# facebookresearch/nonrigid_nerf

Hardware: NVIDIA H100
Metric: rays/sec (64c+128f samples, 8x256 MLP), example_sequence training step (higher is better)
Workload: dtype f16 (tensor-core operands; f32 accumulate)

## Files before the change

include/nrnerf_b200.h:

```cpp
#ifndef NRNERF_B200_H
#define NRNERF_B200_H

#include <stddef.h>
#include <stdint.h>

#ifdef __cplusplus
extern "C" {
#endif

#define NRN_ABI_VERSION 4

#define NRN_OK 0
#define NRN_E_INVALID (-1)
#define NRN_E_CUDA (-2)
#define NRN_E_DEVICE (-3)

int nrn_abi_version(void);
const char* nrn_last_error(void);

int nrn_device_error(int* code_out);

size_t nrn_packed_nerf_bytes(void);
size_t nrn_packed_bender_bytes(void);
int nrn_pack_nerf(const float* const* w, const float* const* b, int input_ch, int out_ch, void* packed,
// ... 23 lines not shown
  const void* nerf_packed;
  const void* bender_packed;
  int32_t out_ch;
  int32_t use_cutoff;  float rigidity_cutoff;
  int32_t use_scaling; float scaling;
  int32_t use_removal; float removal_threshold;
  float* raw;
  float* initial_input_pts;
  float* input_pts;
  float* unmasked_offsets;
  float* masked_offsets;
  float* rigidity_mask;
  void* stash;
  void* stream;
  void* relu_mask;
} NrnFieldArgs;
int nrn_field_forward(const NrnFieldArgs* args);

typedef struct NrnCompositeArgs {
  const float* raw;
  const float* z_vals;
  const float* rays_d;
  int32_t rays_d_stride;
  const float* noise;
  int32_t n_rays, n_samples, channels, white_bkgd;
  float* rgb_map;
  float* disp_map;
  float* acc_map;
  float* depth_map;
  float* weights;
// ... 282 lines not shown
```

nonrigid_nerf_b200/_lib.py:

```python
from __future__ import annotations

import ctypes as C
import os
import threading

_HERE = os.path.dirname(os.path.abspath(__file__))
LIB_PATH = os.path.join(_HERE, "libnrnerf_b200.so")
ABI_VERSION = 4

_f32p = C.POINTER(C.c_float)
_vp = C.c_void_p


class NrnFieldArgs(C.Structure):
    _fields_ = [
        ("rays", _vp), ("z_vals", _vp), ("points", _vp), ("points_stride", C.c_int64),
        ("latents", _vp), ("latent_stride", C.c_int64),
        ("n_rays", C.c_int32), ("n_samples", C.c_int32),
        ("nerf_packed", _vp), ("bender_packed", _vp),
        ("out_ch", C.c_int32),
        ("use_cutoff", C.c_int32), ("rigidity_cutoff", C.c_float),
        ("use_scaling", C.c_int32), ("scaling", C.c_float),
        ("use_removal", C.c_int32), ("removal_threshold", C.c_float),
        ("raw", _vp), ("initial_input_pts", _vp), ("input_pts", _vp), ("unmasked_offsets", _vp),
        ("masked_offsets", _vp), ("rigidity_mask", _vp),
        ("stash", _vp),
        ("stream", _vp),
        ("relu_mask", _vp),
    ]


class NrnViewArgs(C.Structure):
    _fields_ = [
        ("views_packed", _vp), ("viewdirs", _vp), ("viewdirs_stride", C.c_int64), ("workspace", _vp),
    ]


class NrnViewTrainArgs(C.Structure):
    _fields_ = [("views_stash", _vp), ("hv_mask", _vp)]


class NrnViewBwdArgs(C.Structure):
    _fields_ = [("views_t_packed", _vp), ("views_stash", _vp), ("views_grad_stash", _vp), ("hv_mask", _vp)]
# ... 211 lines not shown
    "nrn_lpips": (C.c_int, [C.POINTER(NrnLpipsArgs)]),
    "nrn_timing_enable": (C.c_int, [C.c_int]),
    "nrn_timing_read": (C.c_int, [C.POINTER(C.c_double), C.POINTER(C.c_int), C.c_int]),
}

KERNEL_KINDS = ("field_fwd", "field_dgrad", "wgrad", "composite", "composite_bwd", "divergence")
TC_KERNEL_KINDS = ("tc_latent_bias", "tc_latent_bwd")
VIEW_KERNEL_KINDS = ("views_bend", "views_field")
VIEW_TRAIN_KERNEL_KINDS = ("views_field_train", "views_dgrad", "views_wgrad")
DET_KERNEL_KINDS = ("latent_reduce", "div_loss_reduce")
HELD_OUT_KERNEL_KINDS = ("field_dgrad_held_out", "div_bwd_held_out")
EVAL_KERNEL_KINDS = ("image_scores", "disparity_images", "frame_std_image")
FRAME_IMAGE_KERNEL_KINDS = ("frame_images",)
MESH_KERNEL_KINDS = ("mesh_points", "mesh_count", "mesh_emit", "mesh_colors")
LPIPS_KERNEL_KINDS = ("lpips_input", "lpips_conv", "lpips_pool", "lpips_distance")


def timing_enable(on: bool) -> None:
    check(load().nrn_timing_enable(1 if on else 0), "timing_enable")


def timing_read(kinds=KERNEL_KINDS):
    n = len(kinds)
    ms = (C.c_double * n)()
    cnt = (C.c_int * n)()
    check(load().nrn_timing_read(ms, cnt, n), "timing_read")
    return {k: (ms[i], cnt[i]) for i, k in enumerate(kinds)}

_lib = None
_lock = threading.Lock()
# ... 35 lines not shown
```

nonrigid_nerf_b200/csrc/c_abi.cu:

```cuda
#include <cstdarg>
#include <cstdio>
#include <cstring>
#include <cstdlib>
#include "../../include/nrnerf_b200.h"
#include "nrn_common.cuh"
#include "pack.cuh"
#include "ray_ops.cuh"
#include "wgrad.cuh"
#include "div.cuh"
#include "loss.cuh"
#include "adam.cuh"
#include "peer.cuh"
#include "det_reduce.cuh"
#include "eval.cuh"
#include "mesh.cuh"
#include "lpips.cuh"

namespace nrn {
cudaError_t launch_field_fwd(const FieldFwdParams& p, bool has_bender, int num_sms, cudaStream_t stream);
cudaError_t launch_field_bwd(const FieldBwdParams& p, bool has_bender, int num_sms, cudaStream_t stream);
cudaError_t launch_field_bwd_det(const FieldBwdParams& p, float* latent_rows, int num_sms, cudaStream_t stream);
cudaError_t launch_field_bwd_held(const FieldBwdParams& p, float* latent_rows, const uint8_t* held, int num_sms, cudaStream_t stream);
cudaError_t launch_field_fwd_tc(const FieldFwdParams& p, int num_sms, cudaStream_t stream);
cudaError_t launch_tc_latent_bias(const float* lat, long long lat_stride, int n_rays, const float* w0, const float* b0, const float* w5,
                                  const float* b5, float* rb, cudaStream_t stream);
cudaError_t launch_tc_latent_bwd(const TcBwdParams& p, cudaStream_t stream);
cudaError_t launch_field_bend(const FieldFwdParams& p, const ViewParams& v, int num_sms, cudaStream_t stream);
cudaError_t launch_field_views(const FieldFwdParams& p, const ViewParams& v, int num_sms, cudaStream_t stream);
cudaError_t launch_field_views_train(const FieldFwdParams& p, const ViewParams& v, const ViewTrainParams& t, int num_sms, cudaStream_t stream);
cudaError_t launch_field_bwd_views(const FieldBwdParams& p, const ViewBwdParams& v, int num_sms, cudaStream_t stream);
}

namespace {

thread_local char g_err[512] = "";

int fail(int code, const char* fmt, ...) {
  va_list ap;
  va_start(ap, fmt);
  vsnprintf(g_err, sizeof(g_err), fmt, ap);
  va_end(ap);
  return code;
}
int cuda_fail(cudaError_t e, const char* what) {
  return fail(NRN_E_CUDA, "%s: %s", what, cudaGetErrorString(e));
}

constexpr int kMaxDevices = 64;
struct DeviceState {
  int* err_word = nullptr;
  int num_sms = 0;
};
DeviceState g_dev[kMaxDevices];

int device_state(DeviceState** out) {
  int dev = 0;
  cudaError_t e = cudaGetDevice(&dev);
  if (e != cudaSuccess) return cuda_fail(e, "cudaGetDevice");
  if (dev < 0 || dev >= kMaxDevices) return fail(NRN_E_INVALID, "device index %d out of range", dev);
  DeviceState& s = g_dev[dev];
  if (!s.err_word) {
    cudaDeviceProp prop;
    e = cudaGetDeviceProperties(&prop, dev);
    if (e != cudaSuccess) return cuda_fail(e, "cudaGetDeviceProperties");
    if (prop.major != 9 || prop.minor != 0)
      return fail(NRN_E_INVALID, "nrnerf_b200 is built for sm_90a (H100) only, found sm_%d%d", prop.major, prop.minor);
// ... 241 lines not shown
  if (!pix || !poses || !K || !rays_o || !rays_d || (images && !target)) return fail(NRN_E_INVALID, "nrn_ray_batch: null argument");
  static_assert(sizeof(long long) == sizeof(int64_t), "int64");
  const cudaError_t e = nrn::launch_ray_batch(reinterpret_cast<const long long*>(pix), n, poses, K, image_to_view, images, H, W, rays_o, rays_d,
                                              target, static_cast<cudaStream_t>(stream));
  return e == cudaSuccess ? NRN_OK : cuda_fail(e, "ray_batch_kernel");
}

int nrn_median_visibility_index(const float* weights, int n_rays, int n_samples, int64_t* index, void* stream) {
  if (n_rays < 0 || n_samples < 1) return fail(NRN_E_INVALID, "nrn_median_visibility_index: bad sizes");
  if (n_rays == 0) return NRN_OK;
  if (!weights || !index) return fail(NRN_E_INVALID, "nrn_median_visibility_index: null argument");
  const cudaError_t e = nrn::launch_median_index(weights, n_rays, n_samples, reinterpret_cast<long long*>(index), static_cast<cudaStream_t>(stream));
  return e == cudaSuccess ? NRN_OK : cuda_fail(e, "median_index_kernel");
}

static int field_forward(const NrnFieldArgs* a, const float* ray_bias, const char* who) {
  long long P;
  int tiles;
  int rc = check_field_args(a, who, &P, &tiles);
  if (rc || P == 0) return rc;
  if (!a->raw) return fail(NRN_E_INVALID, "%s: null argument", who);
  if (a->points && a->n_samples != 1) return fail(NRN_E_INVALID, "%s: point mode needs n_samples=1, stride>=3", who);
  DeviceState* ds;
  rc = device_state(&ds);
  if (rc) return rc;
  nrn::FieldFwdParams p = field_fwd_params(a, P, tiles, ds->err_word);
  p.ray_bias = ray_bias; p.ray_bias_stride = a->latent_stride == 0 ? 0 : 2 * 256;
  cudaStream_t st = static_cast<cudaStream_t>(a->stream);
  if (ray_bias) return timed(0, st, "field_fwd_tc_kernel", [&] { return nrn::launch_field_fwd_tc(p, ds->num_sms, st); });
  return timed(0, st, "field_fwd_kernel", [&] { return nrn::launch_field_fwd(p, a->bender_packed != nullptr, ds->num_sms, st); });
}

int nrn_field_forward(const NrnFieldArgs* a) { return field_forward(a, nullptr, "nrn_field_forward"); }

int nrn_field_forward_tc(const NrnFieldArgs* a, const float* ray_bias) {
  if (!a) return fail(NRN_E_INVALID, "nrn_field_forward_tc: null args");
  if (a->bender_packed) return fail(NRN_E_INVALID, "nrn_field_forward_tc: the time-conditioned baseline has no bender (bender_packed must be NULL)");
  if (a->latent_stride < 0) return fail(NRN_E_INVALID, "nrn_field_forward_tc: latent_stride < 0");
  if (a->n_rays > 0 && !ray_bias) return fail(NRN_E_INVALID, "nrn_field_forward_tc: null ray_bias (nrn_tc_latent_bias output)");
  return field_forward(a, ray_bias, "nrn_field_forward_tc");
}

size_t nrn_packed_views_bytes(void) { return nrn::kViewsPackedBytes; }

// ... 36 lines not shown
  if (bend && (!v->workspace || !aligned16(v->workspace)))
    return fail(NRN_E_INVALID, "%s: a bender needs the workspace (nrn_views_workspace_bytes, 16-byte aligned)", who);
  if (v->views_packed && !aligned16(v->views_packed)) return fail(NRN_E_INVALID, "%s: packed weights must be 16-byte aligned", who);
  DeviceState* ds;
  rc = device_state(&ds);
  if (rc) return rc;
  cudaStream_t st = static_cast<cudaStream_t>(a->stream);
  nrn::FieldFwdParams p = field_fwd_params(a, P, tiles, ds->err_word);
  nrn::ViewParams vp{};
  const uint8_t* vw = static_cast<const uint8_t*>(v->views_packed);
  vp.w = vw; vp.bias = vw ? reinterpret_cast<const float*>(vw + nrn::kViewsWBytes) : nullptr;
  vp.viewdirs = v->viewdirs; vp.viewdirs_stride = v->viewdirs_stride;
  if (bend) {
    nrn::FieldFwdParams b = p;
    if (a->points) { b.n_rays = static_cast<int>(P); b.S = 1; }
    vp.ws = static_cast<float4*>(v->workspace);
    rc = timed(8, st, "field_bend_kernel", [&] { return nrn::launch_field_bend(b, vp, ds->num_sms, st); });
    if (rc || !a->raw) return rc;
    p.d_init = p.d_bent = nullptr;
  }
  return timed(9, st, "field_views_kernel", [&] { return nrn::launch_field_views(p, vp, ds->num_sms, st); });
}

size_t nrn_packed_views_t_bytes(void) { return nrn::kViewsTWBytes; }

int nrn_pack_views_t(const float* const* w, void* packed, void* stream) {
  if (!w || !packed) return fail(NRN_E_INVALID, "nrn_pack_views_t: null argument");
  if (!aligned16(packed)) return fail(NRN_E_INVALID, "nrn_pack_views_t: packed buffer must be 16-byte aligned");
  nrn::ViewsSrc src{};
  for (int i = 0; i < 3; ++i) {
    if (!w[i]) return fail(NRN_E_INVALID, "nrn_pack_views_t: null layer %d", i);
    src.w[i] = w[i];
// ... 841 lines not shown
```

nonrigid_nerf_b200/csrc/field_fwd.cu:

```cuda
#include "field_mma.cuh"

namespace nrn {

namespace {

constexpr int kFwdStageLd = 12;
constexpr int kFwdHBytes = kStHb1.chunks * kChunkBytes;
static_assert(kStHb2.chunks <= kStHb1.chunks && kStHb3.chunks <= kStHb1.chunks && kStHb4.chunks <= kStHb1.chunks, "bender images fit H");
constexpr int kFwdRingStages = 5;
constexpr size_t kFwdSmemBytes = kFwdHBytes + kEBytes + kFwdRingStages * kRingStageBytes + 2 * kWgRows * kFwdStageLd * sizeof(float) +
                                 sizeof(RingShared<kFwdRingStages>) + 64;
static_assert(kFwdSmemBytes <= 227 * 1024, "forward kernel: dynamic shared memory per block");

static_assert(fwd::step(fwd::L2) == fwd::step(fwd::L1) && fwd::step(fwd::L3) == fwd::step(fwd::L1) &&
              fwd::step(fwd::L4) == fwd::step(fwd::L1) && fwd::step(fwd::L6) == fwd::step(fwd::L1) &&
              fwd::step(fwd::L7) == fwd::step(fwd::L1), "step_at: one default shape");
__device__ __forceinline__ Step step_at(int step) {
  switch (step) {
    case fwd::B0: return step_imm<fwd::B0>();
    case fwd::B1: return step_imm<fwd::B1>();
    case fwd::B2: return step_imm<fwd::B2>();
    case fwd::B3: return step_imm<fwd::B3>();
    case fwd::B4: return step_imm<fwd::B4>();
    case fwd::L0: return step_imm<fwd::L0>();
    case fwd::L5: return step_imm<fwd::L5>();
    case fwd::Head: return step_imm<fwd::Head>();
    default: return step_imm<fwd::L1>();
  }
}
template <int NCOLS, bool MASK, int NR>
__device__ __forceinline__ void epi_bias_relu_store(const float (&acc)[NR], const float* __restrict__ bias, uint8_t* img, int g,
                                                    uint8_t* mask_tile, int mask_off) {
  const int r0 = g * kWgRows + acc_r0(), q = acc_q();
  ReluMask<NCOLS> m;
  if constexpr (MASK) m.clear();
#pragma unroll
  for (int j = 0; j < NCOLS / 8; ++j) {
    const float2 b = __ldg(reinterpret_cast<const float2*>(bias + 8 * j + 2 * q));
// ... 85 lines not shown
}

static_assert(views::step(views::Feature) == fwd::step(fwd::L1), "step_at_views: Feature has the trunk's shape");
__device__ __forceinline__ Step step_at_views(int step) {
  switch (step) {
    case fwd::L0: return step_imm<fwd::L0>();
    case fwd::L5: return step_imm<fwd::L5>();
    case fwd::Head: return step_imm<fwd::Head>();
    case views::ViewsE: return step_imm<views::ViewsE>();
    case views::ViewsF: return step_imm<views::ViewsF>();
    case views::Rgb: return step_imm<views::Rgb>();
    default: return step_imm<fwd::L1>();
  }
}

enum Part : int { kFull, kBend, kViews };

}

template <bool HAS_BENDER, bool TRAIN, bool LATENT_BIAS, int PART = kFull>
__device__ __forceinline__ void field_fwd_body(const FieldFwdParams& p, const ViewParams& v = ViewParams{},
                                               const ViewTrainParams& t = ViewTrainParams{}) {
  static_assert(!(HAS_BENDER && LATENT_BIAS), "the time-conditioned baseline has no bender");
  static_assert(PART == kFull || (!LATENT_BIAS && (PART == kBend) == HAS_BENDER && (!TRAIN || PART == kViews)),
                "view-head parts: inference, or training of the view-head kernel without a bender");
  constexpr int kHBytes = PART == kViews ? 0 : kFwdHBytes;
  extern __shared__ __align__(1024) uint8_t smem[];
  uint8_t* act = smem;
  uint8_t* ring_buf = smem + kHBytes + kEBytes;
  float* stage_all = reinterpret_cast<float*>(ring_buf + kFwdRingStages * kRingStageBytes);
  auto* sh = reinterpret_cast<RingShared<kFwdRingStages>*>(stage_all + 2 * kWgRows * kFwdStageLd);

  const int warp = threadIdx.x >> 5;
  const int lane = threadIdx.x & 31;

  if (threadIdx.x == 0) sh->init();
  __syncthreads();
  const Waiter W{&sh->abort_flag, p.err};
  Ring<kFwdRingStages> ring{ring_buf, sh->w_full, sh->w_empty};

  if (warp >= 8) {
    setmaxnreg_dec<kProducerRegs>();
    if (warp == 8 && lane == 0) {
      if constexpr (PART == kViews) produce(p.nerf_w, v.w, p.n_tiles, fwd::L0, views::kEnd, views::Feature, step_at_views, ring, W);
      else produce(p.bend_w, p.nerf_w, p.n_tiles, HAS_BENDER ? fwd::B0 : fwd::L0, PART == kBend ? fwd::L0 : fwd::kCount, fwd::L0, step_at, ring, W);
    }
    return;
  }

  setmaxnreg_inc<kConsumerRegs>();
  const int g = warp >> 2;
  const int tw = threadIdx.x & 127;
  const bool row_thread = tw < kWgRows;
  const int bar = 1 + g;
  const bool wg_leader = tw == 0;
  uint8_t* Hs = act;
  uint8_t* Es = act + kHBytes;
  uint8_t* e_row = Es + (g * kWgRows + tw) * 16;
  const uint32_t a_h = smem_u32(Hs) + g * kWgRows * 16;
  const uint32_t a_e = smem_u32(Es) + g * kWgRows * 16;
  float* stg = stage_all + g * kWgRows * kFwdStageLd;
  float* my_stg = stg + tw * kFwdStageLd;

  for (int tile = blockIdx.x; tile < p.n_tiles; tile += gridDim.x) {
    const long long pt = static_cast<long long>(tile) * kTileM + g * kWgRows + tw;
    const bool valid = row_thread && pt < p.P;
    uint8_t* st = p.stash ? p.stash + static_cast<long long>(tile) * kStashTileBytes : nullptr;
    const StashWriter<true> sw{st, wg_leader, bar, g};
    uint8_t* mk = TRAIN ? p.relu_mask + static_cast<long long>(tile) * kMaskTileBytes : nullptr;
    float x[3] = {0.f, 0.f, 0.f};
    long long ray = 0;
    if (valid) {
      ray = pt / p.S;
      if (PART == kViews && v.ws) {
        const float4 q = __ldg(v.ws + pt);
        const bool first = pt % p.S == 0;
        const float4 o = __ldg(v.ws + (first ? pt + 1 : pt - 1));
        x[0] = q.x; x[1] = q.y; x[2] = q.z;
        const float dx = first ? o.x - q.x : q.x - o.x, dy = first ? o.y - q.y : q.y - o.y, dz = first ? o.z - q.z : q.z - o.z;
        const float nrm = __fadd_rn(__fsqrt_rn(__fadd_rn(__fadd_rn(__fmul_rn(dx, dx), __fmul_rn(dy, dy)), __fmul_rn(dz, dz))), 1e-6f);
        my_stg[8] = __fdiv_rn(dx, nrm); my_stg[9] = __fdiv_rn(dy, nrm); my_stg[10] = __fdiv_rn(dz, nrm);
        my_stg[11] = q.w;
      } else if (p.pts) {
        const float* q = p.pts + pt * p.pts_stride;
        x[0] = __ldg(q + 0); x[1] = __ldg(q + 1); x[2] = __ldg(q + 2);
      } else {
        const float z = __ldg(p.z_vals + pt);
        const float* r = p.rays + ray * 8;
        x[0] = __fadd_rn(__ldg(r + 0), __fmul_rn(__ldg(r + 3), z));
        x[1] = __fadd_rn(__ldg(r + 1), __fmul_rn(__ldg(r + 4), z));
        x[2] = __fadd_rn(__ldg(r + 2), __fmul_rn(__ldg(r + 5), z));
      }
      if (PART == kViews && !v.ws) {
        const float* vd = v.viewdirs + (p.pts ? pt : ray) * v.viewdirs_stride;
        my_stg[8] = __ldg(vd + 0); my_stg[9] = __ldg(vd + 1); my_stg[10] = __ldg(vd + 2);
      }
      if (p.d_init) {
        p.d_init[pt * 3 + 0] = x[0]; p.d_init[pt * 3 + 1] = x[1]; p.d_init[pt * 3 + 2] = x[2];
      }
    }
    float rigidity = 0.f;
    if (HAS_BENDER) {
      sw.begin();
      if (row_thread) {
        float in[48];
#pragma unroll
        for (int d = 0; d < 3; ++d) {
          const float hi = __half2float(__float2half_rn(x[d]));
          in[d] = hi;
          in[3 + d] = x[d] - hi;
        }
        const float* lat = p.latents + ray * p.latent_stride;
#pragma unroll
        for (int i = 0; i < kLatent; ++i) in[6 + i] = valid ? __ldg(lat + i) : 0.f;
#pragma unroll
        for (int i = 38; i < 48; ++i) in[i] = 0.f;
        pack_row(in, e_row);
      }
      sw.ready(kStBin, Es);
      {
        Acc<fwd::B0> acc;
        wg_gemm_step<fwd::B0>(acc, ring, [&](uint32_t) { return a_e; }, W, 301);
        sw.begin();
        epi_bias_relu_store<kMkHb1.cols, TRAIN>(acc, p.bend_bias + fwd::b_off(fwd::B0), Hs, g, mk, kMkHb1.off);
        sw.ready(kStHb1, Hs);
        wg_gemm_step<fwd::B1>(acc, ring, [&](uint32_t) { return a_h; }, W, 302);
        sw.begin();
        epi_bias_relu_store<kMkHb2.cols, TRAIN>(acc, p.bend_bias + fwd::b_off(fwd::B1), Hs, g, mk, kMkHb2.off);
        sw.ready(kStHb2, Hs);
      }
      {
        Acc<fwd::B2> acc;
        wg_gemm_step<fwd::B2>(acc, ring, [&](uint32_t) { return a_h; }, W, 303);
        sw.begin();
        epi_bias_relu_store<kMkHb3.cols, TRAIN>(acc, p.bend_bias + fwd::b_off(fwd::B2), Hs, g, mk, kMkHb3.off);
        if (acc_q() == 0) {
          stg[acc_r0() * kFwdStageLd] = acc[32];
          stg[(acc_r0() + 8) * kFwdStageLd] = acc[34];
        }
        sw.ready(kStHb3, Hs);
        if (row_thread) {
          const float rr = my_stg[0] + __ldg(p.bend_bias + fwd::b_off(fwd::B2) + 64);
          rigidity = (tanhf(rr) + 1.0f) * 0.5f;
          if (p.use_cutoff && rigidity <= p.cutoff) rigidity = 0.f;
        }
      }
      {
        Acc<fwd::B3> acc;
        wg_gemm_step<fwd::B3>(acc, ring, [&](uint32_t) { return a_h; }, W, 304);
        sw.begin();
        epi_bias_relu_store<kMkHb4.cols, TRAIN>(acc, p.bend_bias + fwd::b_off(fwd::B3), Hs, g, mk, kMkHb4.off);
        sw.ready(kStHb4, Hs);
      }
      {
        Acc<fwd::B4> acc;
        wg_gemm_step<fwd::B4>(acc, ring, [&](uint32_t) { return a_h; }, W, 305);
        stage_cols<0, 1>(acc, stg, kFwdStageLd);
        wg_bar(bar);
        if (row_thread) {
          float un[3], ma[3];
#pragma unroll
          for (int d = 0; d < 3; ++d) {
            un[d] = my_stg[d];
            ma[d] = __fmul_rn(rigidity, un[d]);
            if (p.use_scaling) ma[d] = __fmul_rn(ma[d], p.scaling);
          }
          if (valid) {
            if (p.d_unmasked) { p.d_unmasked[pt * 3 + 0] = un[0]; p.d_unmasked[pt * 3 + 1] = un[1]; p.d_unmasked[pt * 3 + 2] = un[2]; }
            if (p.d_masked) { p.d_masked[pt * 3 + 0] = ma[0]; p.d_masked[pt * 3 + 1] = ma[1]; p.d_masked[pt * 3 + 2] = ma[2]; }
            if (p.d_rigid) p.d_rigid[pt] = rigidity;
          }
#pragma unroll
          for (int d = 0; d < 3; ++d) x[d] = __fadd_rn(x[d], ma[d]);
        }
      }
    }
    if (valid && p.d_bent) {
      p.d_bent[pt * 3 + 0] = x[0]; p.d_bent[pt * 3 + 1] = x[1]; p.d_bent[pt * 3 + 2] = x[2];
    }
    if constexpr (PART == kBend) {
      if (valid) v.ws[pt] = make_float4(x[0], x[1], x[2], rigidity);
      continue;
    }
    sw.begin();
    if (row_thread) write_pe(x, e_row);
    sw.ready(kStE, Es);
    uint32_t h[kMaskHCols / 16][4];
    int ray_r0 = 0, ray_r8 = 0;
    if constexpr (LATENT_BIAS) {
      const long long r0 = static_cast<long long>(tile) * kTileM + g * kWgRows + acc_r0();
      ray_r0 = static_cast<int>(min(r0, p.P - 1) / p.S);
      ray_r8 = static_cast<int>(min(r0 + 8, p.P - 1) / p.S);
    }
#pragma unroll 1
    for (int L = 0; L < 8; ++L) {
      Acc<fwd::L1> acc;
      if (L == 0) wg_gemm_step<fwd::L0>(acc, ring, [&](uint32_t) { return a_e; }, W, 310);
// ... 6 lines not shown
        epi_bias_frag<kMaskHCols, true, TRAIN>(acc, p.nerf_bias + L * fwd::b_off(fwd::L1), h, st + st_h(L + 1).off, g,
                                               mk + kMkH + L * kMaskHBytes);
      }
    }
    if constexpr (PART == kViews) {
      uint8_t* vst = TRAIN ? t.vstash + static_cast<long long>(tile) * kVStashTileBytes : nullptr;
      const StashWriter<true> vsw{vst, wg_leader, bar, g};
      {
        Acc<fwd::Head> acc;
        wg_gemm_rs<fwd::step(fwd::Head).N, fwd::step(fwd::Head).k16>(acc, h, ring, false, 0u, W, 320);
        stage_cols<0, 1>(acc, stg, kFwdStageLd);
        if constexpr (TRAIN) sw.begin();
        else wg_bar(bar);
        if (row_thread) {
          float alpha = my_stg[3] + __ldg(p.nerf_bias + fwd::b_off(fwd::Head) + 3);
          if (v.ws && p.use_removal && my_stg[11] >= p.removal) alpha *= 0.f;
          const bool dir_ok = !TRAIN || valid;
          const float d[3] = {dir_ok ? my_stg[8] : 0.f, dir_ok ? my_stg[9] : 0.f, dir_ok ? my_stg[10] : 0.f};
          my_stg[11] = alpha;
          write_dir_enc(d, e_row);
        }
      }
      {
        Acc<views::Feature> acc;
        wg_gemm_rs<views::step(views::Feature).N, views::step(views::Feature).k16>(acc, h, ring, false, 0u, W, 330);
        epi_bias_frag<256, false, TRAIN>(acc, v.bias + views::b_off(views::Feature), h, TRAIN ? vst + kVsF.off : nullptr, g);
      }
      if constexpr (TRAIN) {
        vsw.ready(kVsDir, Es);
      } else {
        fence_proxy_async_smem();
// ... 26 lines not shown
      stage_cols<0, 1>(acc, stg, kFwdStageLd);
      wg_bar(bar);
      if (valid) {
        float o[5];
#pragma unroll
        for (int c = 0; c < 5; ++c) o[c] = my_stg[c] + __ldg(p.nerf_bias + fwd::b_off(fwd::Head) + c);
        if (HAS_BENDER && p.use_removal && rigidity >= p.removal) o[3] *= 0.f;
        float* dst = p.raw + pt * p.out_ch;
        for (int c = 0; c < p.out_ch; ++c) dst[c] = o[c];
      }
    }
  }
  if (p.stash && wg_leader) tma_bulk_wait<0>();
}

template <bool HAS_BENDER, bool TRAIN>
__global__ void __launch_bounds__(kFwdThreads, 1) field_fwd_kernel(const FieldFwdParams p) { field_fwd_body<HAS_BENDER, TRAIN, false>(p); }
template <bool TRAIN>
__global__ void __launch_bounds__(kFwdThreads, 1) field_fwd_tc_kernel(const FieldFwdParams p) { field_fwd_body<false, TRAIN, true>(p); }
__global__ void __launch_bounds__(kFwdThreads, 1) field_bend_kernel(const FieldFwdParams p, const ViewParams v) {
  field_fwd_body<true, false, false, kBend>(p, v);
}
__global__ void __launch_bounds__(kFwdThreads, 1) field_views_kernel(const FieldFwdParams p, const ViewParams v) {
  field_fwd_body<false, false, false, kViews>(p, v);
}
__global__ void __launch_bounds__(kFwdThreads, 1) field_views_train_kernel(const FieldFwdParams p, const ViewParams v, const ViewTrainParams t) {
  field_fwd_body<false, true, false, kViews>(p, v, t);
}

constexpr int kTcRaysPerBlock = 16;
__global__ void __launch_bounds__(256) tc_latent_bias_kernel(const float* __restrict__ lat, long long lat_stride, int n_rays,
                                                             const float* __restrict__ w0, const float* __restrict__ b0,
                                                             const float* __restrict__ w5, const float* __restrict__ b5,
                                                             float* __restrict__ rb) {
  __shared__ float zs[kTcRaysPerBlock][kLatent];
  const int o = threadIdx.x;
  const int n0 = blockIdx.x * kTcRaysPerBlock;
// ... 19 lines not shown
    float* dst = rb + static_cast<long long>(n0 + i) * 512;
    dst[o] = ba + sa;
    dst[256 + o] = bb + sb;
  }
}

size_t field_fwd_smem_bytes() { return kFwdSmemBytes; }

cudaError_t launch_field_fwd(const FieldFwdParams& p, bool has_bender, int num_sms, cudaStream_t stream) {
  const size_t smem = field_fwd_smem_bytes();
  const bool train = p.relu_mask != nullptr;
  if (has_bender) return launch_field(train ? field_fwd_kernel<true, true> : field_fwd_kernel<true, false>, p, num_sms, smem, stream);
  return launch_field(train ? field_fwd_kernel<false, true> : field_fwd_kernel<false, false>, p, num_sms, smem, stream);
}

size_t field_views_smem_bytes() { return kFwdSmemBytes - kFwdHBytes; }

cudaError_t launch_field_bend(const FieldFwdParams& p, const ViewParams& v, int num_sms, cudaStream_t stream) {
  return launch_field(field_bend_kernel, p, num_sms, field_fwd_smem_bytes(), stream, v);
}

cudaError_t launch_field_views(const FieldFwdParams& p, const ViewParams& v, int num_sms, cudaStream_t stream) {
  return launch_field(field_views_kernel, p, num_sms, field_views_smem_bytes(), stream, v);
}

cudaError_t launch_field_views_train(const FieldFwdParams& p, const ViewParams& v, const ViewTrainParams& t, int num_sms, cudaStream_t stream) {
  return launch_field(field_views_train_kernel, p, num_sms, field_views_smem_bytes(), stream, v, t);
}

cudaError_t launch_field_fwd_tc(const FieldFwdParams& p, int num_sms, cudaStream_t stream) {
  const bool train = p.relu_mask != nullptr;
  return launch_field(train ? field_fwd_tc_kernel<true> : field_fwd_tc_kernel<false>, p, num_sms, field_fwd_smem_bytes(), stream);
}

cudaError_t launch_tc_latent_bias(const float* lat, long long lat_stride, int n_rays, const float* w0, const float* b0, const float* w5,
                                  const float* b5, float* rb, cudaStream_t stream) {
  tc_latent_bias_kernel<<<(n_rays + kTcRaysPerBlock - 1) / kTcRaysPerBlock, 256, 0, stream>>>(lat, lat_stride, n_rays, w0, b0, w5, b5, rb);
  return cudaGetLastError();
}

}
```

nonrigid_nerf_b200/csrc/nrn_common.cuh:

```cuda
#pragma once
#include <cuda_runtime.h>
#include <stdint.h>

namespace nrn {

constexpr int kTileM = 128;
constexpr int kChunkBytes = kTileM * 16;
constexpr int kRingStageBytes = 32768;
constexpr int kFwdThreads = 384;
constexpr int kProducerRegs = 40, kConsumerRegs = 232;
constexpr int kLatent = 32;

struct WImage {
  int rows, chunks;
  __host__ __device__ constexpr int bytes() const { return rows * chunks * 16; }
  __host__ __device__ constexpr WImage t() const { return {8 * chunks, rows / 8}; }
};

namespace fwd {
enum Id : int { B0, B1, B2, B3, B4, L0, L1, L2, L3, L4, L5, L6, L7, Head, kCount };
__host__ __device__ constexpr WImage image(int s) {
  switch (s) {
    case B0: return {96, 6};
    case B1: return {96, 12};
// ... 206 lines not shown
  const float* bend_bias;
  float cutoff, scaling, removal;
  int use_cutoff, use_scaling, use_removal;
  int out_ch;
  float* raw;
  float* d_init;
  float* d_bent;
  float* d_unmasked;
  float* d_masked;
  float* d_rigid;
  uint8_t* stash;
  int* err;
  uint8_t* relu_mask;
  const float* ray_bias;
  long long ray_bias_stride;
};

struct ViewParams {
  const uint8_t* w;
  const float* bias;
  const float* viewdirs;
  long long viewdirs_stride;
  float4* ws;
};
struct ViewTrainParams {
  uint8_t* vstash;
  uint8_t* hv_mask;
};
struct ViewBwdParams {
  const uint8_t* wT;
  const uint8_t* hv_mask;
  uint8_t* vgstash;
};

struct TcBwdParams {
  const uint8_t* gstash;
  const float* amax;
  long long P;
// ... 12 lines not shown
```

nonrigid_nerf_b200/ops.py:

```python
from __future__ import annotations

import ctypes as C
from typing import Dict, Optional, Tuple

import torch

from . import _lib

LATENT = 32
FORCE_PACK = False


def _ptr(t: Optional[torch.Tensor]):
    return None if t is None else C.c_void_p(t.data_ptr())


def _stream():
    return C.c_void_p(torch.cuda.current_stream().cuda_stream)


def _f32c(t: torch.Tensor, name: str) -> torch.Tensor:
    if not t.is_cuda:
        raise RuntimeError(f"nonrigid_nerf_b200: {name} must be a CUDA tensor (there is no CPU path)")
    if t.dtype != torch.float32:
# ... 219 lines not shown
        viewdirs = viewdirs.reshape(viewdirs.shape[0], -1).float().contiguous().to(dev)
    return viewdirs, viewdirs.stride(0) if viewdirs.shape[0] > 1 else 3


def _field(rays, z_vals, points, latents, nerf_pack, bender_pack, out_ch, cutoff, scaling, removal, want_details, stash=None, relu_mask=None,
           tc_net=None):
    tc = tc_net if bender_pack is None else None
    if latents is None and (bender_pack is not None or tc is not None):
        raise RuntimeError("nonrigid_nerf_b200: " + ("ray bending" if tc is None else "time_conditioned_baseline") + " needs latents")
    a, raw, details, keep = _field_args(rays, z_vals, points, 1, latents if bender_pack is not None or tc is not None else None, nerf_pack,
                                        bender_pack, out_ch, (cutoff, scaling, removal), True, want_details)
    if stash is not None:
        a.stash = stash.data_ptr()
    if relu_mask is not None:
        a.relu_mask = relu_mask.data_ptr()
    with torch.cuda.device(keep[0].device):
        if tc is not None:
            ray_bias = tc_ray_bias(tc, keep[-1], a.latent_stride)
            _lib.check(_lib.load().nrn_field_forward_tc(C.byref(a), _ptr(ray_bias)), "field_forward_tc")
        else:
            _lib.check(_lib.load().nrn_field_forward(C.byref(a)), "field_forward")
    return raw, details


def field_forward(rays: torch.Tensor, z_vals: torch.Tensor, latents: Optional[torch.Tensor], nerf_pack: torch.Tensor,
                  bender_pack: Optional[torch.Tensor], out_ch: int, cutoff: Optional[float] = None,
                  scaling: Optional[float] = None, removal: Optional[float] = None,
                  want_details: bool = False, stash: Optional[torch.Tensor] = None,
                  relu_mask: Optional[torch.Tensor] = None, tc_net=None) -> Tuple[torch.Tensor, Dict[str, torch.Tensor]]:
    return _field(rays, z_vals, None, latents, nerf_pack, bender_pack, out_ch, cutoff, scaling, removal, want_details, stash,
# ... 191 lines not shown
```

Baseline: 492,500.

## Split ray bender into a standalone kernel with smem-resident weights

The forward field kernel used to run the bender MLP inline before the NeRF MLP, streaming bender weights through the shared weight ring and reserving an extra activation buffer. A new dedicated bend kernel now loads all bender weights into shared memory once per CTA via TMA, runs four warpgroups (two tiles per CTA) with double-buffered activation images, and writes bent points and rigidity to a float4 workspace. The main forward kernel then reads that workspace, which frees its H buffer in shared memory. The cost is an extra kernel launch, a global round trip of P float4s, and a workspace allocation on each Python call.

```diff
diff --git a/include/nrnerf_b200.h b/include/nrnerf_b200.h
--- a/include/nrnerf_b200.h
+++ b/include/nrnerf_b200.h
@@ -61,6 +61,7 @@
   void* stash;
   void* stream;
   void* relu_mask;
+  void* workspace;
 } NrnFieldArgs;
 int nrn_field_forward(const NrnFieldArgs* args);
 
diff --git a/nonrigid_nerf_b200/_lib.py b/nonrigid_nerf_b200/_lib.py
--- a/nonrigid_nerf_b200/_lib.py
+++ b/nonrigid_nerf_b200/_lib.py
@@ -26,7 +26,7 @@
         ("masked_offsets", _vp), ("rigidity_mask", _vp),
         ("stash", _vp),
         ("stream", _vp),
-        ("relu_mask", _vp),
+        ("relu_mask", _vp), ("workspace", _vp),
     ]
 
 
@@ -268,6 +268,7 @@
 FRAME_IMAGE_KERNEL_KINDS = ("frame_images",)
 MESH_KERNEL_KINDS = ("mesh_points", "mesh_count", "mesh_emit", "mesh_colors")
 LPIPS_KERNEL_KINDS = ("lpips_input", "lpips_conv", "lpips_pool", "lpips_distance")
+BEND_KERNEL_KINDS = ("field_bend",)
 
 
 def timing_enable(on: bool) -> None:
diff --git a/nonrigid_nerf_b200/csrc/c_abi.cu b/nonrigid_nerf_b200/csrc/c_abi.cu
--- a/nonrigid_nerf_b200/csrc/c_abi.cu
+++ b/nonrigid_nerf_b200/csrc/c_abi.cu
@@ -25,7 +25,7 @@
 cudaError_t launch_tc_latent_bias(const float* lat, long long lat_stride, int n_rays, const float* w0, const float* b0, const float* w5,
                                   const float* b5, float* rb, cudaStream_t stream);
 cudaError_t launch_tc_latent_bwd(const TcBwdParams& p, cudaStream_t stream);
-cudaError_t launch_field_bend(const FieldFwdParams& p, const ViewParams& v, int num_sms, cudaStream_t stream);
+cudaError_t launch_field_bend(const FieldFwdParams& p, int num_sms, cudaStream_t stream);
 cudaError_t launch_field_views(const FieldFwdParams& p, const ViewParams& v, int num_sms, cudaStream_t stream);
 cudaError_t launch_field_views_train(const FieldFwdParams& p, const ViewParams& v, const ViewTrainParams& t, int num_sms, cudaStream_t stream);
 cudaError_t launch_field_bwd_views(const FieldBwdParams& p, const ViewBwdParams& v, int num_sms, cudaStream_t stream);
@@ -50,6 +50,8 @@
 struct DeviceState {
   int* err_word = nullptr;
   int num_sms = 0;
+  void* bend_ws = nullptr;
+  size_t bend_ws_bytes = 0;
 };
 DeviceState g_dev[kMaxDevices];
 
@@ -321,6 +323,32 @@
   return e == cudaSuccess ? NRN_OK : cuda_fail(e, "median_index_kernel");
 }
 
+static int bend_workspace(void* given, long long P, DeviceState* ds, cudaStream_t st, const char* who, float4** out) {
+  if (given) {
+    if (!aligned16(given)) return fail(NRN_E_INVALID, "%s: workspace must be 16-byte aligned", who);
+    *out = static_cast<float4*>(given);
+    return NRN_OK;
+  }
+  const size_t need = static_cast<size_t>(P) * sizeof(float4);
+  if (ds->bend_ws_bytes < need) {
+    cudaStreamCaptureStatus cs = cudaStreamCaptureStatusNone;
+    cudaStreamIsCapturing(st, &cs);
+    if (cs != cudaStreamCaptureStatusNone)
+      return fail(NRN_E_INVALID, "%s: a bender needs a workspace during stream capture (nrn_views_workspace_bytes)", who);
+    if (ds->bend_ws) {
+      const cudaError_t e = cudaFree(ds->bend_ws);
+      if (e != cudaSuccess) return cuda_fail(e, "cudaFree(bend workspace)");
+      ds->bend_ws = nullptr;
+      ds->bend_ws_bytes = 0;
+    }
+    const cudaError_t e = cudaMalloc(&ds->bend_ws, need);
+    if (e != cudaSuccess) return cuda_fail(e, "cudaMalloc(bend workspace)");
+    ds->bend_ws_bytes = need;
+  }
+  *out = static_cast<float4*>(ds->bend_ws);
+  return NRN_OK;
+}
+
 static int field_forward(const NrnFieldArgs* a, const float* ray_bias, const char* who) {
   long long P;
   int tiles;
@@ -335,6 +363,13 @@
   p.ray_bias = ray_bias; p.ray_bias_stride = a->latent_stride == 0 ? 0 : 2 * 256;
   cudaStream_t st = static_cast<cudaStream_t>(a->stream);
   if (ray_bias) return timed(0, st, "field_fwd_tc_kernel", [&] { return nrn::launch_field_fwd_tc(p, ds->num_sms, st); });
+  if (a->bender_packed) {
+    rc = bend_workspace(a->workspace, P, ds, st, who, &p.ws);
+    if (rc) return rc;
+    rc = timed(29, st, "field_bend_kernel", [&] { return nrn::launch_field_bend(p, ds->num_sms, st); });
+    if (rc) return rc;
+    p.d_init = p.d_bent = nullptr;
+  }
   return timed(0, st, "field_fwd_kernel", [&] { return nrn::launch_field_fwd(p, a->bender_packed != nullptr, ds->num_sms, st); });
 }
 
@@ -401,8 +436,8 @@
   if (bend) {
     nrn::FieldFwdParams b = p;
     if (a->points) { b.n_rays = static_cast<int>(P); b.S = 1; }
-    vp.ws = static_cast<float4*>(v->workspace);
-    rc = timed(8, st, "field_bend_kernel", [&] { return nrn::launch_field_bend(b, vp, ds->num_sms, st); });
+    b.ws = p.ws = static_cast<float4*>(v->workspace);
+    rc = timed(8, st, "field_bend_kernel", [&] { return nrn::launch_field_bend(b, ds->num_sms, st); });
     if (rc || !a->raw) return rc;
     p.d_init = p.d_bent = nullptr;
   }
diff --git a/nonrigid_nerf_b200/csrc/field_fwd.cu b/nonrigid_nerf_b200/csrc/field_fwd.cu
--- a/nonrigid_nerf_b200/csrc/field_fwd.cu
+++ b/nonrigid_nerf_b200/csrc/field_fwd.cu
@@ -5,10 +5,8 @@
 namespace {
 
 constexpr int kFwdStageLd = 12;
-constexpr int kFwdHBytes = kStHb1.chunks * kChunkBytes;
-static_assert(kStHb2.chunks <= kStHb1.chunks && kStHb3.chunks <= kStHb1.chunks && kStHb4.chunks <= kStHb1.chunks, "bender images fit H");
 constexpr int kFwdRingStages = 5;
-constexpr size_t kFwdSmemBytes = kFwdHBytes + kEBytes + kFwdRingStages * kRingStageBytes + 2 * kWgRows * kFwdStageLd * sizeof(float) +
+constexpr size_t kFwdSmemBytes = kEBytes + kFwdRingStages * kRingStageBytes + 2 * kWgRows * kFwdStageLd * sizeof(float) +
                                  sizeof(RingShared<kFwdRingStages>) + 64;
 static_assert(kFwdSmemBytes <= 227 * 1024, "forward kernel: dynamic shared memory per block");
 
@@ -17,11 +15,6 @@
               fwd::step(fwd::L7) == fwd::step(fwd::L1), "step_at: one default shape");
 __device__ __forceinline__ Step step_at(int step) {
   switch (step) {
-    case fwd::B0: return step_imm<fwd::B0>();
-    case fwd::B1: return step_imm<fwd::B1>();
-    case fwd::B2: return step_imm<fwd::B2>();
-    case fwd::B3: return step_imm<fwd::B3>();
-    case fwd::B4: return step_imm<fwd::B4>();
     case fwd::L0: return step_imm<fwd::L0>();
     case fwd::L5: return step_imm<fwd::L5>();
     case fwd::Head: return step_imm<fwd::Head>();
@@ -137,7 +130,20 @@
   }
 }
 
-enum Part : int { kFull, kBend, kViews };
+__device__ __forceinline__ void sample_point(const FieldFwdParams& p, long long pt, long long ray, float (&x)[3]) {
+  if (p.pts) {
+    const float* q = p.pts + pt * p.pts_stride;
+    x[0] = __ldg(q + 0); x[1] = __ldg(q + 1); x[2] = __ldg(q + 2);
+  } else {
+    const float z = __ldg(p.z_vals + pt);
+    const float* r = p.rays + ray * 8;
+    x[0] = __fadd_rn(__ldg(r + 0), __fmul_rn(__ldg(r + 3), z));
+    x[1] = __fadd_rn(__ldg(r + 1), __fmul_rn(__ldg(r + 4), z));
+    x[2] = __fadd_rn(__ldg(r + 2), __fmul_rn(__ldg(r + 5), z));
+  }
+}
+
+enum Part : int { kFull, kViews };
 
 }
 
@@ -145,12 +151,10 @@
 __device__ __forceinline__ void field_fwd_body(const FieldFwdParams& p, const ViewParams& v = ViewParams{},
                                                const ViewTrainParams& t = ViewTrainParams{}) {
   static_assert(!(HAS_BENDER && LATENT_BIAS), "the time-conditioned baseline has no bender");
-  static_assert(PART == kFull || (!LATENT_BIAS && (PART == kBend) == HAS_BENDER && (!TRAIN || PART == kViews)),
-                "view-head parts: inference, or training of the view-head kernel without a bender");
-  constexpr int kHBytes = PART == kViews ? 0 : kFwdHBytes;
+  static_assert(PART == kFull || (!LATENT_BIAS && !HAS_BENDER), "view-head kernel: no time conditioning, points from p.ws");
   extern __shared__ __align__(1024) uint8_t smem[];
   uint8_t* act = smem;
-  uint8_t* ring_buf = smem + kHBytes + kEBytes;
+  uint8_t* ring_buf = smem + kEBytes;
   float* stage_all = reinterpret_cast<float*>(ring_buf + kFwdRingStages * kRingStageBytes);
   auto* sh = reinterpret_cast<RingShared<kFwdRingStages>*>(stage_all + 2 * kWgRows * kFwdStageLd);
 
@@ -166,7 +170,7 @@
     setmaxnreg_dec<kProducerRegs>();
     if (warp == 8 && lane == 0) {
       if constexpr (PART == kViews) produce(p.nerf_w, v.w, p.n_tiles, fwd::L0, views::kEnd, views::Feature, step_at_views, ring, W);
-      else produce(p.bend_w, p.nerf_w, p.n_tiles, HAS_BENDER ? fwd::B0 : fwd::L0, PART == kBend ? fwd::L0 : fwd::kCount, fwd::L0, step_at, ring, W);
+      else produce(p.nerf_w, p.nerf_w, p.n_tiles, fwd::L0, fwd::kCount, fwd::L0, step_at, ring, W);
     }
     return;
   }
@@ -177,10 +181,8 @@
   const bool row_thread = tw < kWgRows;
   const int bar = 1 + g;
   const bool wg_leader = tw == 0;
-  uint8_t* Hs = act;
-  uint8_t* Es = act + kHBytes;
+  uint8_t* Es = act;
   uint8_t* e_row = Es + (g * kWgRows + tw) * 16;
-  const uint32_t a_h = smem_u32(Hs) + g * kWgRows * 16;
   const uint32_t a_e = smem_u32(Es) + g * kWgRows * 16;
   float* stg = stage_all + g * kWgRows * kFwdStageLd;
   float* my_stg = stg + tw * kFwdStageLd;
@@ -192,29 +194,27 @@
     const StashWriter<true> sw{st, wg_leader, bar, g};
     uint8_t* mk = TRAIN ? p.relu_mask + static_cast<long long>(tile) * kMaskTileBytes : nullptr;
     float x[3] = {0.f, 0.f, 0.f};
+    float rigidity = 0.f;
     long long ray = 0;
     if (valid) {
       ray = pt / p.S;
-      if (PART == kViews && v.ws) {
-        const float4 q = __ldg(v.ws + pt);
+      if (HAS_BENDER) {
+        const float4 q = __ldg(p.ws + pt);
+        x[0] = q.x; x[1] = q.y; x[2] = q.z;
+        rigidity = q.w;
+      } else if (PART == kViews && p.ws) {
+        const float4 q = __ldg(p.ws + pt);
         const bool first = pt % p.S == 0;
-        const float4 o = __ldg(v.ws + (first ? pt + 1 : pt - 1));
+        const float4 o = __ldg(p.ws + (first ? pt + 1 : pt - 1));
         x[0] = q.x; x[1] = q.y; x[2] = q.z;
         const float dx = first ? o.x - q.x : q.x - o.x, dy = first ? o.y - q.y : q.y - o.y, dz = first ? o.z - q.z : q.z - o.z;
         const float nrm = __fadd_rn(__fsqrt_rn(__fadd_rn(__fadd_rn(__fmul_rn(dx, dx), __fmul_rn(dy, dy)), __fmul_rn(dz, dz))), 1e-6f);
         my_stg[8] = __fdiv_rn(dx, nrm); my_stg[9] = __fdiv_rn(dy, nrm); my_stg[10] = __fdiv_rn(dz, nrm);
         my_stg[11] = q.w;
-      } else if (p.pts) {
-        const float* q = p.pts + pt * p.pts_stride;
-        x[0] = __ldg(q + 0); x[1] = __ldg(q + 1); x[2] = __ldg(q + 2);
       } else {
-        const float z = __ldg(p.z_vals + pt);
-        const float* r = p.rays + ray * 8;
-        x[0] = __fadd_rn(__ldg(r + 0), __fmul_rn(__ldg(r + 3), z));
-        x[1] = __fadd_rn(__ldg(r + 1), __fmul_rn(__ldg(r + 4), z));
-        x[2] = __fadd_rn(__ldg(r + 2), __fmul_rn(__ldg(r + 5), z));
-      }
-      if (PART == kViews && !v.ws) {
+        sample_point(p, pt, ray, x);
+      }
+      if (PART == kViews && !p.ws) {
         const float* vd = v.viewdirs + (p.pts ? pt : ray) * v.viewdirs_stride;
         my_stg[8] = __ldg(vd + 0); my_stg[9] = __ldg(vd + 1); my_stg[10] = __ldg(vd + 2);
       }
@@ -222,88 +222,8 @@
         p.d_init[pt * 3 + 0] = x[0]; p.d_init[pt * 3 + 1] = x[1]; p.d_init[pt * 3 + 2] = x[2];
       }
     }
-    float rigidity = 0.f;
-    if (HAS_BENDER) {
-      sw.begin();
-      if (row_thread) {
-        float in[48];
-#pragma unroll
-        for (int d = 0; d < 3; ++d) {
-          const float hi = __half2float(__float2half_rn(x[d]));
-          in[d] = hi;
-          in[3 + d] = x[d] - hi;
-        }
-        const float* lat = p.latents + ray * p.latent_stride;
-#pragma unroll
-        for (int i = 0; i < kLatent; ++i) in[6 + i] = valid ? __ldg(lat + i) : 0.f;
-#pragma unroll
-        for (int i = 38; i < 48; ++i) in[i] = 0.f;
-        pack_row(in, e_row);
-      }
-      sw.ready(kStBin, Es);
-      {
-        Acc<fwd::B0> acc;
-        wg_gemm_step<fwd::B0>(acc, ring, [&](uint32_t) { return a_e; }, W, 301);
-        sw.begin();
-        epi_bias_relu_store<kMkHb1.cols, TRAIN>(acc, p.bend_bias + fwd::b_off(fwd::B0), Hs, g, mk, kMkHb1.off);
-        sw.ready(kStHb1, Hs);
-        wg_gemm_step<fwd::B1>(acc, ring, [&](uint32_t) { return a_h; }, W, 302);
-        sw.begin();
-        epi_bias_relu_store<kMkHb2.cols, TRAIN>(acc, p.bend_bias + fwd::b_off(fwd::B1), Hs, g, mk, kMkHb2.off);
-        sw.ready(kStHb2, Hs);
-      }
-      {
-        Acc<fwd::B2> acc;
-        wg_gemm_step<fwd::B2>(acc, ring, [&](uint32_t) { return a_h; }, W, 303);
-        sw.begin();
-        epi_bias_relu_store<kMkHb3.cols, TRAIN>(acc, p.bend_bias + fwd::b_off(fwd::B2), Hs, g, mk, kMkHb3.off);
-        if (acc_q() == 0) {
-          stg[acc_r0() * kFwdStageLd] = acc[32];
-          stg[(acc_r0() + 8) * kFwdStageLd] = acc[34];
-        }
-        sw.ready(kStHb3, Hs);
-        if (row_thread) {
-          const float rr = my_stg[0] + __ldg(p.bend_bias + fwd::b_off(fwd::B2) + 64);
-          rigidity = (tanhf(rr) + 1.0f) * 0.5f;
-          if (p.use_cutoff && rigidity <= p.cutoff) rigidity = 0.f;
-        }
-      }
-      {
-        Acc<fwd::B3> acc;
-        wg_gemm_step<fwd::B3>(acc, ring, [&](uint32_t) { return a_h; }, W, 304);
-        sw.begin();
-        epi_bias_relu_store<kMkHb4.cols, TRAIN>(acc, p.bend_bias + fwd::b_off(fwd::B3), Hs, g, mk, kMkHb4.off);
-        sw.ready(kStHb4, Hs);
-      }
-      {
-        Acc<fwd::B4> acc;
-        wg_gemm_step<fwd::B4>(acc, ring, [&](uint32_t) { return a_h; }, W, 305);
-        stage_cols<0, 1>(acc, stg, kFwdStageLd);
-        wg_bar(bar);
-        if (row_thread) {
-          float un[3], ma[3];
-#pragma unroll
-          for (int d = 0; d < 3; ++d) {
-            un[d] = my_stg[d];
-            ma[d] = __fmul_rn(rigidity, un[d]);
-            if (p.use_scaling) ma[d] = __fmul_rn(ma[d], p.scaling);
-          }
-          if (valid) {
-            if (p.d_unmasked) { p.d_unmasked[pt * 3 + 0] = un[0]; p.d_unmasked[pt * 3 + 1] = un[1]; p.d_unmasked[pt * 3 + 2] = un[2]; }
-            if (p.d_masked) { p.d_masked[pt * 3 + 0] = ma[0]; p.d_masked[pt * 3 + 1] = ma[1]; p.d_masked[pt * 3 + 2] = ma[2]; }
-            if (p.d_rigid) p.d_rigid[pt] = rigidity;
-          }
-#pragma unroll
-          for (int d = 0; d < 3; ++d) x[d] = __fadd_rn(x[d], ma[d]);
-        }
-      }
-    }
     if (valid && p.d_bent) {
       p.d_bent[pt * 3 + 0] = x[0]; p.d_bent[pt * 3 + 1] = x[1]; p.d_bent[pt * 3 + 2] = x[2];
-    }
-    if constexpr (PART == kBend) {
-      if (valid) v.ws[pt] = make_float4(x[0], x[1], x[2], rigidity);
-      continue;
     }
     sw.begin();
     if (row_thread) write_pe(x, e_row);
@@ -340,7 +260,7 @@
         else wg_bar(bar);
         if (row_thread) {
           float alpha = my_stg[3] + __ldg(p.nerf_bias + fwd::b_off(fwd::Head) + 3);
-          if (v.ws && p.use_removal && my_stg[11] >= p.removal) alpha *= 0.f;
+          if (p.ws && p.use_removal && my_stg[11] >= p.removal) alpha *= 0.f;
           const bool dir_ok = !TRAIN || valid;
           const float d[3] = {dir_ok ? my_stg[8] : 0.f, dir_ok ? my_stg[9] : 0.f, dir_ok ? my_stg[10] : 0.f};
           my_stg[11] = alpha;
@@ -397,13 +317,194 @@
   if (p.stash && wg_leader) tma_bulk_wait<0>();
 }
 
+namespace {
+constexpr int kBendTilesPerCta = 2;
+constexpr int kBendWgs = 2 * kBendTilesPerCta;
+constexpr int kBendThreads = 128 * kBendWgs;
+constexpr int kBendImgBytes = kStHb1.chunks * kChunkBytes;
+static_assert(kStBin.chunks <= kStHb1.chunks && kStHb2.chunks <= kStHb1.chunks && kStHb3.chunks <= kStHb1.chunks &&
+              kStHb4.chunks <= kStHb1.chunks, "bender images fit the tile image");
+struct BendShared {
+  uint64_t w_full;
+  int abort_flag;
+};
+constexpr size_t kBendSmemBytes = 2 * kBendTilesPerCta * kBendImgBytes + kBendWBytes + kBendWgs * kWgRows * kFwdStageLd * sizeof(float) +
+                                  sizeof(BendShared);
+static_assert(kBendWBytes % 128 == 0, "staging behind the weights stays aligned");
+
+template <bool TRAIN>
+struct BendImages {
+  uint8_t* img;
+  uint8_t* tile;
+  bool leader;
+  int bar, h, cur;
+  __device__ __forceinline__ uint8_t* out() const { return img + cur * kBendImgBytes; }
+  __device__ __forceinline__ uint32_t a() const { return smem_u32(img) + (cur ^ 1) * kBendImgBytes + h * kWgRows * 16; }
+  __device__ __forceinline__ void begin() const {
+    if (TRAIN && leader) tma_bulk_wait_read<1>();
+    wg_bar(bar);
+  }
+  __device__ __forceinline__ void ready(Image im) {
+    fence_proxy_async_smem();
+    wg_bar(bar);
+    if (TRAIN && leader) store_rows(tile + static_cast<uint32_t>(im.off), out(), h, im.chunks);
+    cur ^= 1;
+  }
+};
+
+template <auto S>
+__device__ __forceinline__ void wg_mma_resident(Acc<S>& acc, uint32_t a, const uint8_t* w) {
+  constexpr Step s = step(S);
+  static_assert(s.nslabs == 1, "bender steps: one slab");
+  constexpr int N = s.N;
+  const uint64_t adesc = gmma_desc(a, kChunkBytes, 128);
+  const uint64_t bdesc = gmma_desc(smem_u32(w) + fwd::w_off(S), N * 16, 128);
+#pragma unroll
+  for (int i = 0; i < N / 2; ++i) acc[i] = 0.f;
+  acc_fence(acc);
+  wgmma_fence();
+#pragma unroll 1
+  for (uint32_t k = 0; k < s.k16; ++k)
+    wgmma<N, 0, 0>(acc, gmma_desc_advance(adesc, k * 2 * kChunkBytes), gmma_desc_advance(bdesc, k * 2 * N * 16), k ? 1u : 0u);
+  wgmma_commit();
+  wgmma_wait<0>();
+  acc_fence(acc);
+}
+}
+
+template <bool TRAIN>
+__global__ void __launch_bounds__(kBendThreads, 1) field_bend_kernel(const FieldFwdParams p) {
+  extern __shared__ __align__(1024) uint8_t smem[];
+  const int wg = threadIdx.x >> 7;
+  const int h = wg & 1;
+  uint8_t* img = smem + (wg >> 1) * 2 * kBendImgBytes;
+  uint8_t* wb = smem + 2 * kBendTilesPerCta * kBendImgBytes;
+  float* stage_all = reinterpret_cast<float*>(wb + kBendWBytes);
+  float* stg = stage_all + wg * kWgRows * kFwdStageLd;
+  auto* sh = reinterpret_cast<BendShared*>(stage_all + kBendWgs * kWgRows * kFwdStageLd);
+  if (threadIdx.x == 0) {
+    mbar_init(&sh->w_full, 1);
+    sh->abort_flag = 0;
+    fence_mbar_init();
+  }
+  __syncthreads();
+  if (threadIdx.x == 0) {
+    mbar_arrive_expect_tx(&sh->w_full, kBendWBytes);
+    for (uint32_t off = 0; off < static_cast<uint32_t>(kBendWBytes); off += 16384u)
+      tma_bulk_g2s(wb + off, p.bend_w + off, min(kBendWBytes - off, 16384u), &sh->w_full);
+  }
+  const Waiter W{&sh->abort_flag, p.err};
+
+  const int tw = threadIdx.x & 127;
+  const bool row_thread = tw < kWgRows;
+  const int bar = 1 + wg;
+  const bool wg_leader = tw == 0;
+  const int row_off = (h * kWgRows + tw) * 16;
+  BendImages<TRAIN> im{img, nullptr, wg_leader, bar, h, 0};
+  float* my_stg = stg + tw * kFwdStageLd;
+  bool weights_ready = false;
+
+  for (long long tile = static_cast<long long>(blockIdx.x) * kBendTilesPerCta + (wg >> 1); tile < p.n_tiles;
+       tile += static_cast<long long>(gridDim.x) * kBendTilesPerCta) {
+    const long long pt = tile * kTileM + h * kWgRows + tw;
+    const bool valid = row_thread && pt < p.P;
+    if (TRAIN) im.tile = p.stash + tile * kStashTileBytes;
+    uint8_t* mk = TRAIN ? p.relu_mask + tile * kMaskTileBytes : nullptr;
+    float x[3] = {0.f, 0.f, 0.f};
+    long long ray = 0;
+    if (valid) {
+      ray = pt / p.S;
+      sample_point(p, pt, ray, x);
+      if (p.d_init) {
+        p.d_init[pt * 3 + 0] = x[0]; p.d_init[pt * 3 + 1] = x[1]; p.d_init[pt * 3 + 2] = x[2];
+      }
+    }
+    float rigidity = 0.f;
+    im.begin();
+    if (row_thread) {
+      float in[48];
+#pragma unroll
+      for (int d = 0; d < 3; ++d) {
+        const float hi = __half2float(__float2half_rn(x[d]));
+        in[d] = hi;
+        in[3 + d] = x[d] - hi;
+      }
+      const float* lat = p.latents + ray * p.latent_stride;
+#pragma unroll
+      for (int i = 0; i < kLatent; ++i) in[6 + i] = valid ? __ldg(lat + i) : 0.f;
+#pragma unroll
+      for (int i = 38; i < 48; ++i) in[i] = 0.f;
+      pack_row(in, im.out() + row_off);
+    }
+    im.ready(kStBin);
+    if (!weights_ready) {
+      W.wait(&sh->w_full, 0, 300);
+      weights_ready = true;
+    }
+    {
+      Acc<fwd::B0> acc;
+      wg_mma_resident<fwd::B0>(acc, im.a(), wb);
+      im.begin();
+      epi_bias_relu_store<kMkHb1.cols, TRAIN>(acc, p.bend_bias + fwd::b_off(fwd::B0), im.out(), h, mk, kMkHb1.off);
+      im.ready(kStHb1);
+      wg_mma_resident<fwd::B1>(acc, im.a(), wb);
+      im.begin();
+      epi_bias_relu_store<kMkHb2.cols, TRAIN>(acc, p.bend_bias + fwd::b_off(fwd::B1), im.out(), h, mk, kMkHb2.off);
+      im.ready(kStHb2);
+    }
+    {
+      Acc<fwd::B2> acc;
+      wg_mma_resident<fwd::B2>(acc, im.a(), wb);
+      im.begin();
+      epi_bias_relu_store<kMkHb3.cols, TRAIN>(acc, p.bend_bias + fwd::b_off(fwd::B2), im.out(), h, mk, kMkHb3.off);
+      if (acc_q() == 0) {
+        stg[acc_r0() * kFwdStageLd] = acc[32];
+        stg[(acc_r0() + 8) * kFwdStageLd] = acc[34];
+      }
+      im.ready(kStHb3);
+      if (row_thread) {
+        const float rr = my_stg[0] + __ldg(p.bend_bias + fwd::b_off(fwd::B2) + 64);
+        rigidity = (tanhf(rr) + 1.0f) * 0.5f;
+        if (p.use_cutoff && rigidity <= p.cutoff) rigidity = 0.f;
+      }
+    }
+    {
+      Acc<fwd::B3> acc;
+      wg_mma_resident<fwd::B3>(acc, im.a(), wb);
+      im.begin();
+      epi_bias_relu_store<kMkHb4.cols, TRAIN>(acc, p.bend_bias + fwd::b_off(fwd::B3), im.out(), h, mk, kMkHb4.off);
+      im.ready(kStHb4);
+    }
+    {
+      Acc<fwd::B4> acc;
+      wg_mma_resident<fwd::B4>(acc, im.a(), wb);
+      stage_cols<0, 1>(acc, stg, kFwdStageLd);
+      wg_bar(bar);
+      if (valid) {
+        float un[3], ma[3];
+#pragma unroll
+        for (int d = 0; d < 3; ++d) {
+          un[d] = my_stg[d];
+          ma[d] = __fmul_rn(rigidity, un[d]);
+          if (p.use_scaling) ma[d] = __fmul_rn(ma[d], p.scaling);
+        }
+        if (p.d_unmasked) { p.d_unmasked[pt * 3 + 0] = un[0]; p.d_unmasked[pt * 3 + 1] = un[1]; p.d_unmasked[pt * 3 + 2] = un[2]; }
+        if (p.d_masked) { p.d_masked[pt * 3 + 0] = ma[0]; p.d_masked[pt * 3 + 1] = ma[1]; p.d_masked[pt * 3 + 2] = ma[2]; }
+        if (p.d_rigid) p.d_rigid[pt] = rigidity;
+#pragma unroll
+        for (int d = 0; d < 3; ++d) x[d] = __fadd_rn(x[d], ma[d]);
+        if (p.d_bent) { p.d_bent[pt * 3 + 0] = x[0]; p.d_bent[pt * 3 + 1] = x[1]; p.d_bent[pt * 3 + 2] = x[2]; }
+        p.ws[pt] = make_float4(x[0], x[1], x[2], rigidity);
+      }
+    }
+  }
+  if (TRAIN && wg_leader) tma_bulk_wait<0>();
+}
+
 template <bool HAS_BENDER, bool TRAIN>
 __global__ void __launch_bounds__(kFwdThreads, 1) field_fwd_kernel(const FieldFwdParams p) { field_fwd_body<HAS_BENDER, TRAIN, false>(p); }
 template <bool TRAIN>
 __global__ void __launch_bounds__(kFwdThreads, 1) field_fwd_tc_kernel(const FieldFwdParams p) { field_fwd_body<false, TRAIN, true>(p); }
-__global__ void __launch_bounds__(kFwdThreads, 1) field_bend_kernel(const FieldFwdParams p, const ViewParams v) {
-  field_fwd_body<true, false, false, kBend>(p, v);
-}
 __global__ void __launch_bounds__(kFwdThreads, 1) field_views_kernel(const FieldFwdParams p, const ViewParams v) {
   field_fwd_body<false, false, false, kViews>(p, v);
 }
@@ -453,18 +554,22 @@
   return launch_field(train ? field_fwd_kernel<false, true> : field_fwd_kernel<false, false>, p, num_sms, smem, stream);
 }
 
-size_t field_views_smem_bytes() { return kFwdSmemBytes - kFwdHBytes; }
-
-cudaError_t launch_field_bend(const FieldFwdParams& p, const ViewParams& v, int num_sms, cudaStream_t stream) {
-  return launch_field(field_bend_kernel, p, num_sms, field_fwd_smem_bytes(), stream, v);
+cudaError_t launch_field_bend(const FieldFwdParams& p, int num_sms, cudaStream_t stream) {
+  if (p.n_tiles <= 0) return cudaSuccess;
+  auto kernel = p.relu_mask ? field_bend_kernel<true> : field_bend_kernel<false>;
+  const cudaError_t e = cudaFuncSetAttribute(kernel, cudaFuncAttributeMaxDynamicSharedMemorySize, (int)kBendSmemBytes);
+  if (e != cudaSuccess) return e;
+  const int pairs = (p.n_tiles + kBendTilesPerCta - 1) / kBendTilesPerCta;
+  kernel<<<pairs < num_sms ? pairs : num_sms, kBendThreads, kBendSmemBytes, stream>>>(p);
+  return cudaGetLastError();
 }
 
 cudaError_t launch_field_views(const FieldFwdParams& p, const ViewParams& v, int num_sms, cudaStream_t stream) {
-  return launch_field(field_views_kernel, p, num_sms, field_views_smem_bytes(), stream, v);
+  return launch_field(field_views_kernel, p, num_sms, field_fwd_smem_bytes(), stream, v);
 }
 
 cudaError_t launch_field_views_train(const FieldFwdParams& p, const ViewParams& v, const ViewTrainParams& t, int num_sms, cudaStream_t stream) {
-  return launch_field(field_views_train_kernel, p, num_sms, field_views_smem_bytes(), stream, v, t);
+  return launch_field(field_views_train_kernel, p, num_sms, field_fwd_smem_bytes(), stream, v, t);
 }
 
 cudaError_t launch_field_fwd_tc(const FieldFwdParams& p, int num_sms, cudaStream_t stream) {
diff --git a/nonrigid_nerf_b200/csrc/nrn_common.cuh b/nonrigid_nerf_b200/csrc/nrn_common.cuh
--- a/nonrigid_nerf_b200/csrc/nrn_common.cuh
+++ b/nonrigid_nerf_b200/csrc/nrn_common.cuh
@@ -244,6 +244,7 @@
   uint8_t* relu_mask;
   const float* ray_bias;
   long long ray_bias_stride;
+  float4* ws;
 };
 
 struct ViewParams {
@@ -251,7 +252,6 @@
   const float* bias;
   const float* viewdirs;
   long long viewdirs_stride;
-  float4* ws;
 };
 struct ViewTrainParams {
   uint8_t* vstash;
diff --git a/nonrigid_nerf_b200/ops.py b/nonrigid_nerf_b200/ops.py
--- a/nonrigid_nerf_b200/ops.py
+++ b/nonrigid_nerf_b200/ops.py
@@ -257,6 +257,10 @@
         a.stash = stash.data_ptr()
     if relu_mask is not None:
         a.relu_mask = relu_mask.data_ptr()
+    if bender_pack is not None:
+        ws = torch.empty(_lib.load().nrn_views_workspace_bytes(a.n_rays, a.n_samples), dtype=torch.uint8, device=keep[0].device)
+        a.workspace = ws.data_ptr()
+        keep.append(ws)
     with torch.cuda.device(keep[0].device):
         if tc is not None:
             ray_bias = tc_ray_bias(tc, keep[-1], a.latent_stride)
```

New measurement: 502,100 (median of 6 runs). +2.0%, better.
